# omahs/celestia-app

Hardware: AMD Instinct MI355X
Metric: EDS+DAH squares/sec (k=128) (higher is better)
Workload: dtype u8; 1 GPU; k=128 ODS -> EDS + 4k NMT roots + DAH, batch replay; k=128, field=GF(2^8), parallelism=batch1, input_layout=ODS in Q0 of the EDS buffer (placed by the upload), batches_in_flight=4

## Files before the change

### celestia-app_amd/csrc/nmt_device.hpp

```cpp
#pragma once
#include <hip/hip_runtime.h>

#include "cel_internal.hpp"
#include "sha256_device.hpp"

namespace cel {

__device__ __forceinline__ void load_node(const uint32_t* p, uint32_t (&n)[kNodeWords]) {
  const uint4* q = reinterpret_cast<const uint4*>(p);
#pragma unroll
  for (int i = 0; i < 6; i++) {
    const uint4 v = q[i];
    n[4 * i] = v.x; n[4 * i + 1] = v.y; n[4 * i + 2] = v.z; n[4 * i + 3] = v.w;
  }
}

__device__ __forceinline__ void store_node(uint32_t* p, const uint32_t (&n)[kNodeWords]) {
  uint4* q = reinterpret_cast<uint4*>(p);
#pragma unroll
  for (int i = 0; i < 6; i++) q[i] = make_uint4(n[4 * i], n[4 * i + 1], n[4 * i + 2], n[4 * i + 3]);
}

__device__ __forceinline__ void put_digest(uint32_t (&nd)[kNodeWords], const uint32_t (&st)[8]) {
  uint32_t sw[8];
#pragma unroll
  for (int i = 0; i < 8; i++) sw[i] = bswap32(st[i]);
  nd[14] = (nd[14] & 0xFFFFu) | (sw[0] << 16);
#pragma unroll
  for (int i = 15; i <= 21; i++) nd[i] = __builtin_amdgcn_alignbyte(sw[i - 14], sw[i - 15], 2);
  nd[22] = sw[7] >> 16;
  nd[23] = 0;
}


constexpr uint32_t kLeafParPrefix[7] = {0x00FFFFFFu, 0xFFFFFFFFu, 0xFFFFFFFFu, 0xFFFFFFFFu,
                                        0xFFFFFFFFu, 0xFFFFFFFFu, 0xFFFFFFFFu};
constexpr ShaMid kLeafParMid = sha_midstate(kLeafParPrefix, 7);

template <bool PF>
__device__ __forceinline__ void leaf_hash(uint32_t (&st)[8], const uint32_t* __restrict__ sh, bool q0) {
  sha256_init(st);
  uint32_t w[16];
  uint32_t nx[17];
  auto load17 = [&](int b) {
    const uint32_t* base = sh + 16 * b - 8;
    const uint4* p4 = reinterpret_cast<const uint4*>(base);
#pragma unroll
    for (int i = 0; i < 4; i++) {
      const uint4 v = p4[i];
      nx[4 * i] = v.x; nx[4 * i + 1] = v.y; nx[4 * i + 2] = v.z; nx[4 * i + 3] = v.w;
    }
    nx[16] = base[16];
  };
  {
    uint32_t s[9];
    const uint4* p4 = reinterpret_cast<const uint4*>(sh);
    const uint4 v0 = p4[0], v1 = p4[1];
    s[0] = v0.x; s[1] = v0.y; s[2] = v0.z; s[3] = v0.w; s[4] = v1.x; s[5] = v1.y; s[6] = v1.z; s[7] = v1.w;
    s[8] = sh[8];
    if (PF) load17(1);
#pragma unroll
    for (int i = 8; i < 16; i++) w[i] = perm(s[i - 8], s[i - 7], 0x06070001u);
    if (__all(!q0)) {
#pragma unroll
      for (int i = 0; i < 7; i++) w[i] = kLeafParPrefix[i];
      w[7] = 0xFFFF0000u | perm(0u, s[0], 0x0C0C0001u);
      sha256_compress_from<7>(st, mid_regs(kLeafParMid), w);
    } else {
      if (q0) {
        w[0] = perm(0u, s[0], 0x0C000102u);
#pragma unroll
        for (int i = 1; i < 7; i++) w[i] = perm(s[i - 1], s[i], 0x07000102u);
        w[7] = perm(s[6], s[7], 0x07000C0Cu) | perm(0u, s[0], 0x0C0C0001u);
      } else {
#pragma unroll
        for (int i = 0; i < 7; i++) w[i] = kLeafParPrefix[i];
        w[7] = 0xFFFF0000u | perm(0u, s[0], 0x0C0C0001u);
      }
      sha256_compress(st, w);
    }
  }
#pragma unroll 1
  for (int b = 1; b < 8; b++) {
    if (!PF) load17(b);
#pragma unroll
    for (int i = 0; i < 16; i++) w[i] = perm(nx[i], nx[i + 1], 0x06070001u);
    if (PF) {
      if (b < 7) {
        load17(b + 1);
      } else {
        const uint4* p4 = reinterpret_cast<const uint4*>(sh + 120);
        const uint4 v0 = p4[0], v1 = p4[1];
        nx[0] = v0.x; nx[1] = v0.y; nx[2] = v0.z; nx[3] = v0.w; nx[4] = v1.x; nx[5] = v1.y; nx[6] = v1.z; nx[7] = v1.w;
      }
    }
    sha256_compress(st, w);
  }
  {
    if (!PF) {
      const uint4* p4 = reinterpret_cast<const uint4*>(sh + 120);
      const uint4 v0 = p4[0], v1 = p4[1];
      nx[0] = v0.x; nx[1] = v0.y; nx[2] = v0.z; nx[3] = v0.w; nx[4] = v1.x; nx[5] = v1.y; nx[6] = v1.z; nx[7] = v1.w;
    }
#pragma unroll
    for (int i = 0; i < 7; i++) w[i] = perm(nx[i], nx[i + 1], 0x06070001u);
    w[7] = perm(nx[7], 0x80u, 0x0607000Cu);
#pragma unroll
    for (int i = 8; i < 15; i++) w[i] = 0u;
    w[15] = 542u * 8u;
    sha256_compress(st, w);
  }
}

__device__ __forceinline__ void leaf_record(const uint32_t* __restrict__ sh, bool q0, const uint32_t (&st)[8],
                                            uint32_t (&nd)[kNodeWords]) {
  if (q0) {
    const uint4* p4 = reinterpret_cast<const uint4*>(sh);
    uint32_t s[8];
    const uint4 v0 = p4[0], v1 = p4[1];
    s[0] = v0.x; s[1] = v0.y; s[2] = v0.z; s[3] = v0.w; s[4] = v1.x; s[5] = v1.y; s[6] = v1.z; s[7] = v1.w;
#pragma unroll
    for (int i = 0; i < 7; i++) nd[i] = s[i];
    nd[7] = (s[7] & 0xFFu) | (s[0] << 8);
#pragma unroll
    for (int i = 0; i < 6; i++) nd[8 + i] = __builtin_amdgcn_alignbyte(s[i + 1], s[i], 3);
    nd[14] = (s[6] >> 24) | ((s[7] & 0xFFu) << 8);
  } else {
#pragma unroll
    for (int i = 0; i < 14; i++) nd[i] = 0xFFFFFFFFu;
    nd[14] = 0xFFFFu;
  }
  put_digest(nd, st);
}

template <bool PF>
__device__ __forceinline__ void make_leaf_node(const uint32_t* __restrict__ sh, bool q0, uint32_t (&nd)[kNodeWords]) {
  uint32_t st[8];
  leaf_hash<PF>(st, sh, q0);
  leaf_record(sh, q0, st, nd);
}

__device__ __forceinline__ bool ns_less(const uint32_t* __restrict__ a, const uint32_t* __restrict__ b) {
  const uint4* pa = reinterpret_cast<const uint4*>(a);
  const uint4* pb = reinterpret_cast<const uint4*>(b);
  uint32_t x[8], y[8];
#pragma unroll
  for (int i = 0; i < 2; i++) {
    const uint4 u = pa[i], v = pb[i];
    x[4 * i] = u.x; x[4 * i + 1] = u.y; x[4 * i + 2] = u.z; x[4 * i + 3] = u.w;
    y[4 * i] = v.x; y[4 * i + 1] = v.y; y[4 * i + 2] = v.z; y[4 * i + 3] = v.w;
  }
  int res = 0;
#pragma unroll
  for (int i = 0; i < 8; i++) {
    uint32_t xa = bswap32(x[i]), yb = bswap32(y[i]);
    if (i == 7) { xa &= 0xFF000000u; yb &= 0xFF000000u; }
    if (res == 0 && xa != yb) res = xa < yb ? -1 : 1;
  }
  return res < 0;
}

__device__ __forceinline__ bool min_is_parity(const uint32_t* __restrict__ R) {
  bool par = (R[7] & 0xFFu) == 0xFFu;
#pragma unroll
  for (int q = 0; q < 7; q++) par = par && (R[q] == 0xFFFFFFFFu);
  return par;
}


constexpr uint32_t kNodeParPrefix[14] = {0x01FFFFFFu, 0xFFFFFFFFu, 0xFFFFFFFFu, 0xFFFFFFFFu, 0xFFFFFFFFu,
                                         0xFFFFFFFFu, 0xFFFFFFFFu, 0xFFFFFFFFu, 0xFFFFFFFFu, 0xFFFFFFFFu,
                                         0xFFFFFFFFu, 0xFFFFFFFFu, 0xFFFFFFFFu, 0xFFFFFFFFu};
constexpr ShaMid kNodeParMid = sha_midstate(kNodeParPrefix, 14);

__device__ __forceinline__ uint32_t node_word(const uint32_t (&L)[kNodeWords], const uint32_t (&R)[kNodeWords], int q) {
  if (q == 0) return perm(1u, L[0], 0x04000102u);
  if (q <= 21) return perm(L[q - 1], L[q], 0x07000102u);
  if (q == 22) return perm(L[21], L[22], 0x0700010Cu) | (R[0] & 0xFFu);
  if (q <= 44) return perm(R[q - 23], R[q - 22], 0x05060700u);
  if (q == 45) return perm(R[22], 0x80u, 0x05000C0Cu);
  if (q == 47) return 181u * 8u;
  return 0u;
}

__device__ __forceinline__ void hash_node(const uint32_t (&L)[kNodeWords], const uint32_t (&R)[kNodeWords],
                                          uint32_t (&out)[kNodeWords]) {
  uint32_t st[8];
  sha256_init(st);
  bool lpar = (L[14] & 0xFFFFu) == 0xFFFFu;
#pragma unroll
  for (int i = 0; i < 14; i++) lpar = lpar && (L[i] == 0xFFFFFFFFu);
  {
    uint32_t w[16];
    if (__all(lpar)) {
#pragma unroll
      for (int wi = 0; wi < 14; wi++) w[wi] = kNodeParPrefix[wi];
      w[14] = node_word(L, R, 14);
      w[15] = node_word(L, R, 15);
      sha256_compress_from<14>(st, mid_regs(kNodeParMid), w);
    } else {
#pragma unroll
      for (int wi = 0; wi < 16; wi++) w[wi] = node_word(L, R, wi);
      sha256_compress(st, w);
    }
  }
#pragma unroll
  for (int b = 1; b < 3; b++) {
    uint32_t w[16];
#pragma unroll
    for (int wi = 0; wi < 16; wi++) w[wi] = node_word(L, R, 16 * b + wi);
    sha256_compress(st, w);
  }
  bool rpar = (R[7] & 0xFFu) == 0xFFu;
#pragma unroll
  for (int i = 0; i < 7; i++) rpar = rpar && (R[i] == 0xFFFFFFFFu);
#pragma unroll
  for (int i = 0; i < 7; i++) out[i] = L[i];
  const uint32_t X7 = rpar ? L[7] : R[7];
  out[7] = (L[7] & 0xFFu) | (X7 & 0xFFFFFF00u);
#pragma unroll
  for (int i = 8; i < 14; i++) out[i] = rpar ? L[i] : R[i];
  out[14] = (rpar ? L[14] : R[14]) & 0xFFFFu;
  put_digest(out, st);
}

__device__ __forceinline__ void hash_pair(const uint32_t* in, uint64_t li, uint64_t ri, uint32_t (&o)[kNodeWords]) {
  uint32_t L[kNodeWords], R[kNodeWords];
  load_node(in + li * kNodeWords, L);
  load_node(in + ri * kNodeWords, R);
  hash_node(L, R, o);
}


constexpr uint32_t kParNodeWords[48] = {
    0x01FFFFFFu, 0xFFFFFFFFu, 0xFFFFFFFFu, 0xFFFFFFFFu, 0xFFFFFFFFu, 0xFFFFFFFFu, 0xFFFFFFFFu, 0xFFFFFFFFu,
    0xFFFFFFFFu, 0xFFFFFFFFu, 0xFFFFFFFFu, 0xFFFFFFFFu, 0xFFFFFFFFu, 0xFFFFFFFFu, 0xFFFFFF00u, 0x00000000u,
    0x00000000u, 0x00000000u, 0x00000000u, 0x00000000u, 0x00000000u, 0x00000000u, 0x000000FFu, 0xFFFFFFFFu,
    0xFFFFFFFFu, 0xFFFFFFFFu, 0xFFFFFFFFu, 0xFFFFFFFFu, 0xFFFFFFFFu, 0xFFFFFFFFu, 0xFFFFFFFFu, 0xFFFFFFFFu,
    0xFFFFFFFFu, 0xFFFFFFFFu, 0xFFFFFFFFu, 0xFFFFFFFFu, 0xFFFFFFFFu, 0xFF000000u, 0x00000000u, 0x00000000u,
    0x00000000u, 0x00000000u, 0x00000000u, 0x00000000u, 0x00000000u, 0x00800000u, 0x00000000u, 181u * 8u};

template <bool COMPACT>
__device__ __forceinline__ void hash_parity_node(const uint32_t (&dl)[8], const uint32_t (&dr)[8],
                                                 uint32_t (&out)[8]) {
  constexpr int kEnd = COMPACT ? 32 : 64;
  uint32_t st[8], w[16];
  sha256_init(st);
  auto finish = [&](ShaRegs& r) {
    if (COMPACT) sha256_rounds_tail(r, w);
    sha256_add(st, r);
  };
  {
#pragma unroll
    for (int i = 0; i < 14; i++) w[i] = kParNodeWords[i];
    w[14] = kParNodeWords[14] | (dl[0] >> 24);
    w[15] = __builtin_amdgcn_alignbit(dl[0], dl[1], 24);
    ShaRegs r = mid_regs(kNodeParMid);
    sha256_rounds_folded<14, kEnd>(r, w);
    finish(r);
  }
  {
#pragma unroll
    for (int i = 0; i < 6; i++) w[i] = __builtin_amdgcn_alignbit(dl[i + 1], dl[i + 2], 24);
    w[6] = kParNodeWords[22] | (dl[7] << 8);
#pragma unroll
    for (int i = 7; i < 16; i++) w[i] = kParNodeWords[16 + i];
    ShaRegs r{st[0], st[1], st[2], st[3], st[4], st[5], st[6], st[7]};
    sha256_rounds_folded<0, kEnd>(r, w);
    finish(r);
  }
  {
#pragma unroll
    for (int i = 0; i < 5; i++) w[i] = kParNodeWords[32 + i];
    w[5] = kParNodeWords[37] | (dr[0] >> 8);
#pragma unroll
    for (int i = 6; i < 13; i++) w[i] = __builtin_amdgcn_alignbit(dr[i - 6], dr[i - 5], 8);
    w[13] = kParNodeWords[45] | (dr[7] << 24);
    w[14] = kParNodeWords[46];
    w[15] = kParNodeWords[47];
    ShaRegs r{st[0], st[1], st[2], st[3], st[4], st[5], st[6], st[7]};
    sha256_rounds_folded<0, kEnd>(r, w);
    finish(r);
  }
#pragma unroll
  for (int i = 0; i < 8; i++) out[i] = st[i];
}

__device__ __forceinline__ void parity_record(const uint32_t (&d)[8], uint32_t (&nd)[kNodeWords]) {
#pragma unroll
  for (int i = 0; i < 14; i++) nd[i] = 0xFFFFFFFFu;
  nd[14] = 0xFFFFu;
  put_digest(nd, d);
}

__device__ __forceinline__ void load_digest(const uint32_t* p, uint32_t (&d)[8]) {
  const uint4* q = reinterpret_cast<const uint4*>(p);
  const uint4 a = q[0], b = q[1];
  d[0] = a.x; d[1] = a.y; d[2] = a.z; d[3] = a.w; d[4] = b.x; d[5] = b.y; d[6] = b.z; d[7] = b.w;
}

__device__ __forceinline__ void store_digest(uint32_t* p, const uint32_t (&d)[8]) {
  uint4* q = reinterpret_cast<uint4*>(p);
  q[0] = make_uint4(d[0], d[1], d[2], d[3]);
  q[1] = make_uint4(d[4], d[5], d[6], d[7]);
}


__device__ __forceinline__ void sha_empty(uint32_t (&st)[8]) {
  uint32_t w[16];
  w[0] = 0x80000000u;
#pragma unroll
  for (int i = 1; i < 16; i++) w[i] = 0;
  sha256_init(st);
  sha256_compress(st, w);
}

__device__ __forceinline__ void rfc_leaf90(const uint32_t (&R)[kNodeWords], uint32_t (&st)[8]) {
  sha256_init(st);
#pragma unroll
  for (int b = 0; b < 2; b++) {
    uint32_t w[16];
#pragma unroll
    for (int wi = 0; wi < 16; wi++) {
      const int q = 16 * b + wi;
      uint32_t x;
      if (q == 0) x = perm(0u, R[0], 0x0C000102u);
      else if (q <= 21) x = perm(R[q - 1], R[q], 0x07000102u);
      else if (q == 22) x = perm(R[21], R[22], 0x0700010Cu) | 0x80u;
      else if (q == 31) x = 91u * 8u;
      else x = 0u;
      w[wi] = x;
    }
    sha256_compress(st, w);
  }
}

__device__ __forceinline__ void rfc_inner(const uint32_t* l, const uint32_t* r, uint32_t (&st)[8]) {
  uint32_t w[16];
  w[0] = 0x01000000u | (l[0] >> 8);
#pragma unroll
  for (int i = 1; i < 8; i++) w[i] = __builtin_amdgcn_alignbit(l[i - 1], l[i], 8);
  w[8] = __builtin_amdgcn_alignbit(l[7], r[0], 8);
#pragma unroll
  for (int i = 9; i < 16; i++) w[i] = __builtin_amdgcn_alignbit(r[i - 9], r[i - 8], 8);
  sha256_init(st);
  uint32_t w2[16];
  w2[0] = (r[7] << 24) | 0x00800000u;
#pragma unroll
  for (int i = 1; i < 15; i++) w2[i] = 0;
  w2[15] = 65u * 8u;
  sha256_compress(st, w);
  sha256_compress(st, w2);
}

}
```

### celestia-app_amd/csrc/nmt_kernels.hip

```cpp
#include <hip/hip_runtime.h>

#include <climits>

#include "cel_internal.hpp"
#include "nmt_device.hpp"
#include "nmt_host.hpp"
#include "sha256_device.hpp"

namespace cel {




template <bool ORDER, bool PF>
__global__ __launch_bounds__(256) void k_leaf(const uint8_t* __restrict__ eds, uint32_t k, uint32_t* __restrict__ leaves,
                                              int32_t* __restrict__ bad_axis, uint32_t cell0, uint32_t cell1) {
  const uint32_t W = 2 * k;
  const uint32_t cell = cell0 + blockIdx.x * 256u + threadIdx.x;
  if (cell >= cell1) return;
  const uint32_t r = cell / W, c = cell % W;
  const uint64_t sq_eds = (uint64_t)W * W * kShare;
  const uint32_t* sh = reinterpret_cast<const uint32_t*>(eds + blockIdx.y * sq_eds + (uint64_t)cell * kShare);
  const bool q0 = (r < k) && (c < k);
  {
    uint32_t nd[kNodeWords];
    make_leaf_node<PF>(sh, q0, nd);
    store_node(leaves + ((uint64_t)blockIdx.y * W * W + cell) * kNodeWords, nd);
  }
  __builtin_amdgcn_sched_barrier(0);
  if (ORDER && q0) {
    if (c > 0 && ns_less(sh, sh - kShare / 4)) atomicMin(bad_axis + blockIdx.y, (int32_t)r);
    if (r > 0 && ns_less(sh, sh - (uint64_t)W * kShare / 4)) atomicMin(bad_axis + blockIdx.y, (int32_t)(W + c));
  }
}


__device__ __forceinline__ void put_root(const uint32_t (&o)[kNodeWords], uint32_t sq, uint32_t t, uint32_t W,
                                         uint32_t* __restrict__ leafd, uint8_t* __restrict__ row_out,
                                         uint8_t* __restrict__ col_out) {
  {
    uint8_t* r = (t < W ? row_out + ((uint64_t)sq * W + t) * kNode : col_out + ((uint64_t)sq * W + (t - W)) * kNode);
    uint16_t* r16 = reinterpret_cast<uint16_t*>(r);
#pragma unroll
    for (int i = 0; i < 45; i++) r16[i] = (uint16_t)(o[i / 2] >> (16 * (i & 1)));
  }
  if (leafd) {
    uint32_t st[8];
    rfc_leaf90(o, st);
    uint4* d = reinterpret_cast<uint4*>(leafd + ((uint64_t)sq * 2 * W + t) * 8);
    d[0] = make_uint4(st[0], st[1], st[2], st[3]);
    d[1] = make_uint4(st[4], st[5], st[6], st[7]);
  }
}

template <bool FROM_LEAVES>
__global__ __launch_bounds__(256) void k_level(const uint32_t* __restrict__ in, uint32_t* __restrict__ out, uint32_t W,
                                               uint32_t nin, uint32_t trees, uint32_t* __restrict__ leafd,
                                               uint8_t* __restrict__ row_out, uint8_t* __restrict__ col_out) {
  const uint32_t nout = nin / 2;
  const uint32_t idx = blockIdx.x * 256u + threadIdx.x;
  if (idx >= trees * nout) return;
  const uint32_t t = idx / nout, j = idx % nout;
  uint64_t li, ri;
  if (FROM_LEAVES) {
    const uint64_t sq = (uint64_t)blockIdx.y * W * W;
    if (t < W) { li = sq + (uint64_t)t * W + 2 * j; ri = li + 1; }
    else { li = sq + (uint64_t)(2 * j) * W + (t - W); ri = li + W; }
  } else {
    const uint64_t sq = (uint64_t)blockIdx.y * trees * nin;
    li = sq + (uint64_t)t * nin + 2 * j;
    ri = li + 1;
  }
  uint32_t o[kNodeWords];
  hash_pair(in, li, ri, o);
  const uint64_t oi = (uint64_t)blockIdx.y * trees * nout + idx;
  store_node(out + oi * kNodeWords, o);
  if (row_out) put_root(o, blockIdx.y, t, W, leafd, row_out, col_out);
}


__host__ __device__ constexpr uint32_t q_nodes(uint32_t k, uint32_t n) { return k * n; }
__host__ __device__ constexpr uint32_t p_nodes(uint32_t k, uint32_t n) { return 3 * k * n; }
__device__ __forceinline__ uint32_t q_node(uint32_t k, uint32_t n, uint32_t t, uint32_t i) {
  return (t < k ? t : t - k) * (n / 2) + i;
}
__device__ __forceinline__ uint32_t p_node(uint32_t k, uint32_t n, uint32_t t, uint32_t i) {
  const uint32_t W = 2 * k, a = t < W ? t : t - W;
  if (a < k) return (t < W ? a : k + a) * (n / 2) + (i - n / 2);
  return k * n + (t < W ? a - k : a) * n + i;
}

template <bool ROOT>
__global__ __launch_bounds__(256) void k_level_split(const uint32_t* __restrict__ qin, uint32_t* __restrict__ qout,
                                                     const uint32_t* __restrict__ pin, uint32_t* __restrict__ pout,
                                                     uint32_t nq, uint32_t np, uint32_t bq, uint32_t k,
                                                     uint32_t* __restrict__ leafd, uint8_t* __restrict__ row_out,
                                                     uint8_t* __restrict__ col_out) {
  const uint32_t sq = blockIdx.y, W = 2 * k;
  if (blockIdx.x < bq) {
    const uint32_t i = blockIdx.x * 256u + threadIdx.x;
    if (i >= nq) return;
    uint32_t o[kNodeWords];
    if (ROOT) {
      uint32_t L[kNodeWords], R[kNodeWords], d[8];
      load_node(qin + ((uint64_t)sq * nq + i) * kNodeWords, L);
      load_digest(pin + ((uint64_t)sq * 3 * np + i) * 8, d);
      parity_record(d, R);
      hash_node(L, R, o);
      put_root(o, sq, i < k ? i : W + (i - k), W, leafd, row_out, col_out);
    } else {
      hash_pair(qin + (uint64_t)sq * 2 * nq * kNodeWords, 2 * i, 2 * i + 1, o);
      store_node(qout + ((uint64_t)sq * nq + i) * kNodeWords, o);
    }
  } else {
    const uint32_t i = (blockIdx.x - bq) * 256u + threadIdx.x;
    if (i >= np) return;
    const uint32_t* in = pin + (ROOT ? (uint64_t)sq * 3 * np + np : (uint64_t)sq * 2 * np) * 8;
    uint32_t dl[8], dr[8], d[8];
    load_digest(in + (uint64_t)i * 16, dl);
    load_digest(in + (uint64_t)i * 16 + 8, dr);
    hash_parity_node<false>(dl, dr, d);
    if (ROOT) {
      uint32_t o[kNodeWords];
      parity_record(d, o);
      put_root(o, sq, i < k ? k + i : W + i, W, leafd, row_out, col_out);
    } else {
      store_digest(pout + ((uint64_t)sq * np + i) * 8, d);
    }
  }
}


template <bool ORDER, bool PF, bool ROOTS>
__global__ __launch_bounds__(256) __attribute__((amdgpu_waves_per_eu(3, 3))) void k_leaf_quad(
    const uint8_t* __restrict__ eds, uint32_t k, uint32_t* __restrict__ out, uint32_t* __restrict__ pout,
    int32_t* __restrict__ bad_axis, uint32_t* __restrict__ leafd, uint8_t* __restrict__ row_out,
    uint8_t* __restrict__ col_out) {
  const uint32_t W = 2 * k, trees = 2 * W;
  const uint32_t tw = k < 8 ? k : 8u, th = 64 / tw, tiles_x = k / tw;
  const uint32_t g = blockIdx.x * 256u + threadIdx.x, tile = g / 64, l = g % 64;
  const uint32_t bi = (tile / tiles_x) * th + l / tw, bj = (tile % tiles_x) * tw + l % tw;
  if (bi >= k) return;
  const uint64_t sq_eds = (uint64_t)W * W * kShare;
  const uint32_t* sh00 =
      reinterpret_cast<const uint32_t*>(eds + blockIdx.y * sq_eds + ((uint64_t)(2 * bi) * W + 2 * bj) * kShare);
  uint32_t dA[8], dB[8], dC[8];
#pragma unroll 1
  for (uint32_t s = 0; s < 4; s++) {
    const uint32_t r = 2 * bi + (s >> 1), c = 2 * bj + (s & 1);
    const uint32_t* sh = sh00 + ((uint64_t)(s >> 1) * W + (s & 1)) * (kShare / 4);
    const bool q0 = (r < k) && (c < k);
    {
      uint32_t st[8];
      leaf_hash<PF>(st, sh, q0);
#pragma unroll
      for (int i = 0; i < 8; i++) {
        if (s == 0 || s == 3) dA[i] = st[i];
        if (s == 1) dB[i] = st[i];
        if (s == 2) dC[i] = st[i];
      }
    }
    const uint32_t nn = s == 3 ? 2u : (s ? 1u : 0u);
#pragma unroll 1
    for (uint32_t n = 0; n < nn; n++) {
      const uint32_t lc = s < 3 ? 0u : 1u + n;
      const bool row = (s == 1) || (s == 3 && n == 1);
      const uint32_t* shl = sh00 + ((uint64_t)(lc >> 1) * W + (lc & 1)) * (kShare / 4);
      const bool q0l = (2 * bi + (lc >> 1) < k) && (2 * bj + (lc & 1) < k);
      const uint32_t t = row ? r : W + c, idx = row ? bj : bi;
      auto children = [&](uint32_t (&dl)[8], uint32_t (&dr)[8]) {
#pragma unroll
        for (int i = 0; i < 8; i++) {
          dl[i] = lc == 0 ? dA[i] : (lc == 1 ? dB[i] : dC[i]);
          dr[i] = s == 1 ? dB[i] : (s == 2 ? dC[i] : dA[i]);
        }
      };
      if (ROOTS || q0l) {
        uint32_t o[kNodeWords];
        {
          uint32_t L[kNodeWords], R[kNodeWords], dl[8], dr[8];
          children(dl, dr);
          leaf_record(shl, q0l, dl, L);
          leaf_record(sh, q0, dr, R);
          hash_node(L, R, o);
        }
        if (ROOTS) {
          store_node(out + (((uint64_t)blockIdx.y * trees + t) * k + idx) * kNodeWords, o);
          put_root(o, blockIdx.y, t, W, leafd, row_out, col_out);
        } else {
          store_node(out + ((uint64_t)blockIdx.y * q_nodes(k, k) + q_node(k, k, t, idx)) * kNodeWords, o);
        }
      } else {
        uint32_t dl[8], dr[8], o[8];
        children(dl, dr);
        hash_parity_node<true>(dl, dr, o);
        store_digest(pout + ((uint64_t)blockIdx.y * p_nodes(k, k) + p_node(k, k, t, idx)) * 8, o);
      }
    }
    __builtin_amdgcn_sched_barrier(0);
    if (ORDER && q0) {
      if (c > 0 && ns_less(sh, sh - kShare / 4)) atomicMin(bad_axis + blockIdx.y, (int32_t)r);
      if (r > 0 && ns_less(sh, sh - (uint64_t)W * kShare / 4)) atomicMin(bad_axis + blockIdx.y, (int32_t)(W + c));
    }
  }
}



__global__ __launch_bounds__(1024) void k_merkle(const uint32_t* __restrict__ items, const uint32_t* __restrict__ leafd,
                                                uint32_t n, uint8_t* dah, const int32_t* __restrict__ bad_axis,
                                                int32_t* status, const uint8_t* out_src,
                                                uint8_t* __restrict__ host_out, uint32_t out_bytes) {
  extern __shared__ __attribute__((aligned(16))) uint32_t hs[];
  const uint32_t g = blockIdx.x;
  const uint32_t* it = items + (uint64_t)g * n * kNodeWords;
  if (leafd) {
    for (uint32_t i = threadIdx.x; i < n * 8; i += blockDim.x) hs[i] = leafd[(uint64_t)g * n * 8 + i];
  } else {
    for (uint32_t i = threadIdx.x; i < n; i += blockDim.x) {
      uint32_t R[kNodeWords], st[8];
      load_node(it + (uint64_t)i * kNodeWords, R);
      rfc_leaf90(R, st);
#pragma unroll
      for (int j = 0; j < 8; j++) hs[i * 8 + j] = st[j];
    }
  }
  __syncthreads();
  uint32_t cnt = n;
  while (cnt > 1) {
    const uint32_t half = cnt / 2;
    uint32_t st[8];
    for (uint32_t base = 0; base < half; base += blockDim.x) {
      const uint32_t i = base + threadIdx.x;
      if (i < half) rfc_inner(hs + (2 * i) * 8, hs + (2 * i + 1) * 8, st);
      __syncthreads();
      if (i < half) {
#pragma unroll
        for (int j = 0; j < 8; j++) hs[i * 8 + j] = st[j];
      }
      __syncthreads();
    }
    if (cnt & 1) {
      if (threadIdx.x < 8) hs[half * 8 + threadIdx.x] = hs[(cnt - 1) * 8 + threadIdx.x];
      __syncthreads();
    }
    cnt = half + (cnt & 1);
  }
  if (threadIdx.x == 0) {
    uint32_t st[8];
    if (n == 0) sha_empty(st);
    else
      for (int j = 0; j < 8; j++) st[j] = hs[j];
    for (int j = 0; j < 8; j++) {
      dah[g * 32 + 4 * j] = (uint8_t)(st[j] >> 24);
      dah[g * 32 + 4 * j + 1] = (uint8_t)(st[j] >> 16);
      dah[g * 32 + 4 * j + 2] = (uint8_t)(st[j] >> 8);
      dah[g * 32 + 4 * j + 3] = (uint8_t)st[j];
    }
    if (status) status[g] = (bad_axis && bad_axis[g] != INT_MAX) ? CEL_EORDER : CEL_OK;
  }
  if (host_out) {
    __threadfence();
    __syncthreads();
    const uint4* src = reinterpret_cast<const uint4*>(out_src);
    uint4* dst = reinterpret_cast<uint4*>(host_out);
    for (uint32_t i = threadIdx.x; i < out_bytes / 16; i += blockDim.x) dst[i] = src[i];
  }
}

static uint32_t merkle_block(uint32_t n) {
  const uint32_t pairs = ((n / 2 + 63) / 64) * 64;
  return pairs < 64 ? 64u : (pairs > 1024 ? 1024u : pairs);
}

__global__ __launch_bounds__(256) void k_dah_leaves(const uint32_t* __restrict__ items, uint32_t n,
                                                    uint32_t* __restrict__ leafd, uint8_t* __restrict__ row_out,
                                                    uint8_t* __restrict__ col_out) {
  const uint32_t i = blockIdx.x * 256u + threadIdx.x;
  if (i >= n) return;
  uint32_t R[kNodeWords], st[8];
  load_node(items + (uint64_t)i * kNodeWords, R);
  rfc_leaf90(R, st);
  uint4* d = reinterpret_cast<uint4*>(leafd + (uint64_t)i * 8);
  d[0] = make_uint4(st[0], st[1], st[2], st[3]);
  d[1] = make_uint4(st[4], st[5], st[6], st[7]);
  const uint32_t half = n / 2;
  uint16_t* r16 = reinterpret_cast<uint16_t*>(i < half ? row_out + (uint64_t)i * kNode : col_out + (uint64_t)(i - half) * kNode);
#pragma unroll
  for (int j = 0; j < 45; j++) r16[j] = (uint16_t)(R[j / 2] >> (16 * (j & 1)));
}

__global__ void k_fill_i32(int32_t* p, uint32_t n, int32_t v) {
  const uint32_t i = blockIdx.x * blockDim.x + threadIdx.x;
  if (i < n) p[i] = v;
}


void launch_fill_i32(int32_t* p, uint32_t n, int32_t v, uint32_t block, hipStream_t s) {
  hipLaunchKernelGGL(k_fill_i32, dim3((n + block - 1) / block), dim3(block), 0, s, p, n, v);
}

void launch_dah_leaves(const uint32_t* items, uint32_t n, uint32_t* leafd, uint8_t* row_out, uint8_t* col_out,
                       hipStream_t s) {
  hipLaunchKernelGGL(k_dah_leaves, dim3((n + 255) / 256), dim3(256), 0, s, items, n, leafd, row_out, col_out);
}

void launch_merkle(const uint32_t* items, const uint32_t* leafd, uint32_t n, uint32_t lists, uint8_t* dah,
                   const int32_t* bad_axis, int32_t* status, hipStream_t s, const uint8_t* out_src, uint8_t* host_out,
                   uint32_t out_bytes) {
  const size_t lds = (size_t)(n ? n : 1) * 8 * 4;
  hipLaunchKernelGGL(k_merkle, dim3(lists), dim3(merkle_block(n)), lds, s, items, leafd, n, dah, bad_axis, status,
                     out_src, host_out, out_bytes);
}

struct CommitWork {
  uint32_t *leaves, *ping, *pong, *roots, *leafd;
  uint32_t *q[2], *p[2];
  int32_t* bad;
  size_t size;
};

static bool quad_path(uint32_t nsq) { return nsq > 1; }

static CommitWork commit_work(void* work, uint32_t k, uint32_t nsq) {
  const size_t W = 2 * (size_t)k, nb = kNodeWords * 4;
  Carver c(work);
  CommitWork w;
  w.leaves = c.take<uint32_t>(quad_path(nsq) ? 0 : nsq * W * W * nb);
  w.ping = c.take<uint32_t>(nsq * 2 * W * (W / 2 + 1) * nb);
  w.pong = c.take<uint32_t>(nsq * 2 * W * (W / 4 + 1) * nb);
  w.roots = c.take<uint32_t>(nsq * 2 * W * nb);
  w.bad = c.take<int32_t>((size_t)nsq * 4 + 4);
  w.leafd = c.take<uint32_t>(nsq * 2 * W * 32);
  w.size = c.size();
  for (uint32_t i = 0; i < 2; i++) {
    Carver a(i ? w.pong : w.ping);
    w.q[i] = a.take<uint32_t>((size_t)nsq * q_nodes(k, k >> i) * nb);
    w.p[i] = a.take<uint32_t>((size_t)nsq * p_nodes(k, k >> i) * 32);
  }
  return w;
}

size_t nmt_workspace_size(uint32_t k, uint32_t nsq) { return commit_work(nullptr, k, nsq).size; }

hipError_t launch_commit_leaves(const uint8_t* eds, uint32_t k, uint32_t nsq, void* work, bool order_check,
                                uint32_t row0, uint32_t row1, bool init_bad, hipStream_t s) {
  if (quad_path(nsq)) return hipErrorInvalidValue;
  const uint32_t W = 2 * k;
  const CommitWork w = commit_work(work, k, nsq);
  const Range r("nmt.leaf");
  if (init_bad) launch_fill_i32(w.bad, nsq, INT_MAX, 256, s);
  const uint32_t c0 = row0 * W, c1 = row1 * W;
  if (c1 <= c0) return hipGetLastError();
  dim3 gl((c1 - c0 + 255) / 256, nsq);
  dispatch_order_pf(order_check, latency_bound((uint64_t)(c1 - c0) * nsq), [&](auto order, auto pf) {
    hipLaunchKernelGGL((k_leaf<decltype(order)::value, decltype(pf)::value>), gl, dim3(256), 0, s, eds, k, w.leaves,
                       w.bad, c0, c1);
  });
  return hipGetLastError();
}

static hipError_t commit_dah(const CommitWork& w, uint32_t k, uint32_t nsq, uint8_t* row_roots, uint8_t* dah,
                             int32_t* status, hipStream_t s, uint8_t* host_out, uint32_t out_bytes) {
  const Range r("dah");
  if (dah)
    launch_merkle(w.roots, w.leafd, 4 * k, nsq, dah, w.bad, status, s, host_out ? row_roots : nullptr, host_out,
                  out_bytes);
  return hipGetLastError();
}

static hipError_t commit_levels(const CommitWork& w, uint32_t k, uint32_t nsq, uint8_t* row_roots,
                                uint8_t* col_roots, uint8_t* dah, int32_t* status, hipStream_t s, uint8_t* host_out,
                                uint32_t out_bytes) {
  const uint32_t W = 2 * k;
  const uint32_t trees = 2 * W;
  uint32_t nin = W;
  const uint32_t* src = w.leaves;
  uint32_t* dst = w.ping;
  bool first = true;
  roctxRangePushA("nmt.levels");
  while (nin > 1) {
    const uint32_t nout = nin / 2;
    uint32_t* out = (nout == 1) ? w.roots : dst;
    uint32_t* ld = (nout == 1 && dah) ? w.leafd : nullptr;
    dim3 g((trees * nout + 255) / 256, nsq);
    uint8_t* ro = (nout == 1) ? row_roots : nullptr;
    uint8_t* co = (nout == 1) ? col_roots : nullptr;
    if (first) hipLaunchKernelGGL(k_level<true>, g, dim3(256), 0, s, src, out, W, nin, trees, ld, ro, co);
    else hipLaunchKernelGGL(k_level<false>, g, dim3(256), 0, s, src, out, W, nin, trees, ld, ro, co);
    first = false;
    src = out;
    dst = (dst == w.ping) ? w.pong : w.ping;
    nin = nout;
  }
  roctxRangePop();
  return commit_dah(w, k, nsq, row_roots, dah, status, s, host_out, out_bytes);
}

hipError_t launch_commit_trees(uint32_t k, uint32_t nsq, uint8_t* row_roots, uint8_t* col_roots, uint8_t* dah,
                               int32_t* status, void* work, hipStream_t s, uint8_t* host_out, uint32_t out_bytes) {
  if (quad_path(nsq)) return hipErrorInvalidValue;
  return commit_levels(commit_work(work, k, nsq), k, nsq, row_roots, col_roots, dah, status, s, host_out, out_bytes);
}

static hipError_t launch_commit_quads(const uint8_t* eds, uint32_t k, uint32_t nsq, const CommitWork& w,
                                      bool order_check, uint8_t* row_roots, uint8_t* col_roots, bool want_dah,
                                      hipStream_t s) {
  const Range r("nmt.leaf");
  launch_fill_i32(w.bad, nsq, INT_MAX, 256, s);
  const uint32_t tw = k < 8 ? k : 8u, th = 64 / tw;
  const uint64_t lanes = (uint64_t)((k + th - 1) / th) * (k / tw) * 64;
  dim3 g((uint32_t)((lanes + 255) / 256), nsq);
  if (k == 1) {
    uint32_t* ld = want_dah ? w.leafd : nullptr;
    if (order_check)
      hipLaunchKernelGGL((k_leaf_quad<true, false, true>), g, dim3(256), 0, s, eds, k, w.roots, nullptr, w.bad, ld,
                         row_roots, col_roots);
    else
      hipLaunchKernelGGL((k_leaf_quad<false, false, true>), g, dim3(256), 0, s, eds, k, w.roots, nullptr, w.bad, ld,
                         row_roots, col_roots);
    return hipGetLastError();
  }
  dispatch_order_pf(order_check, latency_bound(lanes * nsq), [&](auto order, auto pf) {
    hipLaunchKernelGGL((k_leaf_quad<decltype(order)::value, decltype(pf)::value, false>), g, dim3(256), 0, s, eds, k,
                       w.q[0], w.p[0], w.bad, nullptr, nullptr, nullptr);
  });
  return hipGetLastError();
}

static hipError_t commit_levels_split(const CommitWork& w, uint32_t k, uint32_t nsq, uint8_t* row_roots,
                                      uint8_t* col_roots, bool want_dah, hipStream_t s) {
  const Range r("nmt.levels");
  uint32_t at = 0;
  for (uint32_t n = k; n > 2; n /= 2, at ^= 1) {
    const uint32_t nq = q_nodes(k, n / 2), np = p_nodes(k, n / 2), bq = (nq + 255) / 256;
    hipLaunchKernelGGL(k_level_split<false>, dim3(bq + (np + 255) / 256, nsq), dim3(256), 0, s, w.q[at], w.q[at ^ 1],
                       w.p[at], w.p[at ^ 1], nq, np, bq, k, nullptr, nullptr, nullptr);
  }
  const uint32_t nr = 2 * k, bq = (nr + 255) / 256;
  hipLaunchKernelGGL(k_level_split<true>, dim3(2 * bq, nsq), dim3(256), 0, s, w.q[at], nullptr, w.p[at], nullptr, nr,
                     nr, bq, k, want_dah ? w.leafd : nullptr, row_roots, col_roots);
  return hipGetLastError();
}

hipError_t launch_commit(const uint8_t* eds, uint32_t k, uint32_t nsq, uint8_t* row_roots, uint8_t* col_roots,
                         uint8_t* dah, int32_t* status, void* work, bool order_check, hipStream_t s) {
  if (!quad_path(nsq)) {
    hipError_t e = launch_commit_leaves(eds, k, nsq, work, order_check, 0, 2 * k, true, s);
    if (e == hipSuccess) e = launch_commit_trees(k, nsq, row_roots, col_roots, dah, status, work, s);
    return e;
  }
  const CommitWork w = commit_work(work, k, nsq);
  hipError_t e = launch_commit_quads(eds, k, nsq, w, order_check, row_roots, col_roots, dah != nullptr, s);
  if (e == hipSuccess && k > 1) e = commit_levels_split(w, k, nsq, row_roots, col_roots, dah != nullptr, s);
  if (e == hipSuccess) e = commit_dah(w, k, nsq, row_roots, dah, status, s, nullptr, 0);
  return e;
}


}
```

Baseline: 22990 squares/s.

## Split leaf-quad kernel into Q0-only and parity-only launches with specialized hashing

The leaf-level quad kernel is split into two launches. One covers only Q0 tiles, the other only the parity tiles, so each lane's cell type is known at compile time. This removes the per-lane q0 checks and the wave-wide __all votes on parity prefixes, and lets parity blocks always use the precomputed SHA midstate. The cost is an extra kernel launch and code duplication; small k keeps the old path.

```diff
diff --git a/celestia-app_amd/csrc/nmt_device.hpp b/celestia-app_amd/csrc/nmt_device.hpp
--- a/celestia-app_amd/csrc/nmt_device.hpp
+++ b/celestia-app_amd/csrc/nmt_device.hpp
@@ -37,8 +37,11 @@
                                         0xFFFFFFFFu, 0xFFFFFFFFu, 0xFFFFFFFFu};
 constexpr ShaMid kLeafParMid = sha_midstate(kLeafParPrefix, 7);
 
-template <bool PF>
+enum class Cells { kAny, kQ0, kParity };
+
+template <bool PF, Cells C = Cells::kAny>
 __device__ __forceinline__ void leaf_hash(uint32_t (&st)[8], const uint32_t* __restrict__ sh, bool q0) {
+  if (C != Cells::kAny) q0 = C == Cells::kQ0;
   sha256_init(st);
   uint32_t w[16];
   uint32_t nx[17];
@@ -61,7 +64,7 @@
     if (PF) load17(1);
 #pragma unroll
     for (int i = 8; i < 16; i++) w[i] = perm(s[i - 8], s[i - 7], 0x06070001u);
-    if (__all(!q0)) {
+    if (C == Cells::kParity || (C == Cells::kAny && __all(!q0))) {
 #pragma unroll
       for (int i = 0; i < 7; i++) w[i] = kLeafParPrefix[i];
       w[7] = 0xFFFF0000u | perm(0u, s[0], 0x0C0C0001u);
@@ -183,16 +186,17 @@
   return 0u;
 }
 
+template <bool PAR_START = true>
 __device__ __forceinline__ void hash_node(const uint32_t (&L)[kNodeWords], const uint32_t (&R)[kNodeWords],
                                           uint32_t (&out)[kNodeWords]) {
   uint32_t st[8];
   sha256_init(st);
-  bool lpar = (L[14] & 0xFFFFu) == 0xFFFFu;
+  bool lpar = PAR_START && (L[14] & 0xFFFFu) == 0xFFFFu;
 #pragma unroll
   for (int i = 0; i < 14; i++) lpar = lpar && (L[i] == 0xFFFFFFFFu);
   {
     uint32_t w[16];
-    if (__all(lpar)) {
+    if (PAR_START && __all(lpar)) {
 #pragma unroll
       for (int wi = 0; wi < 14; wi++) w[wi] = kNodeParPrefix[wi];
       w[14] = node_word(L, R, 14);
diff --git a/celestia-app_amd/csrc/nmt_kernels.hip b/celestia-app_amd/csrc/nmt_kernels.hip
--- a/celestia-app_amd/csrc/nmt_kernels.hip
+++ b/celestia-app_amd/csrc/nmt_kernels.hip
@@ -5,6 +5,7 @@
 #include "cel_internal.hpp"
 #include "nmt_device.hpp"
 #include "nmt_host.hpp"
+#include "quad_tiles.hpp"
 #include "sha256_device.hpp"
 
 namespace cel {
@@ -131,28 +132,26 @@
 }
 
 
-template <bool ORDER, bool PF, bool ROOTS>
-__global__ __launch_bounds__(256) __attribute__((amdgpu_waves_per_eu(3, 3))) void k_leaf_quad(
-    const uint8_t* __restrict__ eds, uint32_t k, uint32_t* __restrict__ out, uint32_t* __restrict__ pout,
-    int32_t* __restrict__ bad_axis, uint32_t* __restrict__ leafd, uint8_t* __restrict__ row_out,
-    uint8_t* __restrict__ col_out) {
+template <Cells C, bool ORDER, bool PF, bool ROOTS>
+__device__ __forceinline__ void quad_block(const uint8_t* __restrict__ eds, uint32_t k, uint32_t sq, uint32_t bi,
+                                           uint32_t bj, uint32_t* __restrict__ out, uint32_t* __restrict__ pout,
+                                           int32_t* __restrict__ bad_axis, uint32_t* __restrict__ leafd,
+                                           uint8_t* __restrict__ row_out, uint8_t* __restrict__ col_out) {
+  static_assert(C == Cells::kAny || !ROOTS, "the roots case is a mixed block");
   const uint32_t W = 2 * k, trees = 2 * W;
-  const uint32_t tw = k < 8 ? k : 8u, th = 64 / tw, tiles_x = k / tw;
-  const uint32_t g = blockIdx.x * 256u + threadIdx.x, tile = g / 64, l = g % 64;
-  const uint32_t bi = (tile / tiles_x) * th + l / tw, bj = (tile % tiles_x) * tw + l % tw;
-  if (bi >= k) return;
   const uint64_t sq_eds = (uint64_t)W * W * kShare;
   const uint32_t* sh00 =
-      reinterpret_cast<const uint32_t*>(eds + blockIdx.y * sq_eds + ((uint64_t)(2 * bi) * W + 2 * bj) * kShare);
+      reinterpret_cast<const uint32_t*>(eds + sq * sq_eds + ((uint64_t)(2 * bi) * W + 2 * bj) * kShare);
+  auto in_q0 = [&](uint32_t r, uint32_t c) { return C == Cells::kAny ? (r < k) && (c < k) : C == Cells::kQ0; };
   uint32_t dA[8], dB[8], dC[8];
 #pragma unroll 1
   for (uint32_t s = 0; s < 4; s++) {
     const uint32_t r = 2 * bi + (s >> 1), c = 2 * bj + (s & 1);
     const uint32_t* sh = sh00 + ((uint64_t)(s >> 1) * W + (s & 1)) * (kShare / 4);
-    const bool q0 = (r < k) && (c < k);
+    const bool q0 = in_q0(r, c);
     {
       uint32_t st[8];
-      leaf_hash<PF>(st, sh, q0);
+      leaf_hash<PF, C>(st, sh, q0);
 #pragma unroll
       for (int i = 0; i < 8; i++) {
         if (s == 0 || s == 3) dA[i] = st[i];
@@ -166,7 +165,7 @@
       const uint32_t lc = s < 3 ? 0u : 1u + n;
       const bool row = (s == 1) || (s == 3 && n == 1);
       const uint32_t* shl = sh00 + ((uint64_t)(lc >> 1) * W + (lc & 1)) * (kShare / 4);
-      const bool q0l = (2 * bi + (lc >> 1) < k) && (2 * bj + (lc & 1) < k);
+      const bool q0l = in_q0(2 * bi + (lc >> 1), 2 * bj + (lc & 1));
       const uint32_t t = row ? r : W + c, idx = row ? bj : bi;
       auto children = [&](uint32_t (&dl)[8], uint32_t (&dr)[8]) {
 #pragma unroll
@@ -182,27 +181,63 @@
           children(dl, dr);
           leaf_record(shl, q0l, dl, L);
           leaf_record(sh, q0, dr, R);
-          hash_node(L, R, o);
+          hash_node<C == Cells::kAny>(L, R, o);
         }
         if (ROOTS) {
-          store_node(out + (((uint64_t)blockIdx.y * trees + t) * k + idx) * kNodeWords, o);
-          put_root(o, blockIdx.y, t, W, leafd, row_out, col_out);
+          store_node(out + (((uint64_t)sq * trees + t) * k + idx) * kNodeWords, o);
+          put_root(o, sq, t, W, leafd, row_out, col_out);
         } else {
-          store_node(out + ((uint64_t)blockIdx.y * q_nodes(k, k) + q_node(k, k, t, idx)) * kNodeWords, o);
+          store_node(out + ((uint64_t)sq * q_nodes(k, k) + q_node(k, k, t, idx)) * kNodeWords, o);
         }
       } else {
         uint32_t dl[8], dr[8], o[8];
         children(dl, dr);
-        hash_parity_node<true>(dl, dr, o);
-        store_digest(pout + ((uint64_t)blockIdx.y * p_nodes(k, k) + p_node(k, k, t, idx)) * 8, o);
+        hash_parity_node<C == Cells::kAny>(dl, dr, o);
+        store_digest(pout + ((uint64_t)sq * p_nodes(k, k) + p_node(k, k, t, idx)) * 8, o);
       }
     }
     __builtin_amdgcn_sched_barrier(0);
     if (ORDER && q0) {
-      if (c > 0 && ns_less(sh, sh - kShare / 4)) atomicMin(bad_axis + blockIdx.y, (int32_t)r);
-      if (r > 0 && ns_less(sh, sh - (uint64_t)W * kShare / 4)) atomicMin(bad_axis + blockIdx.y, (int32_t)(W + c));
-    }
-  }
+      if (c > 0 && ns_less(sh, sh - kShare / 4)) atomicMin(bad_axis + sq, (int32_t)r);
+      if (r > 0 && ns_less(sh, sh - (uint64_t)W * kShare / 4)) atomicMin(bad_axis + sq, (int32_t)(W + c));
+    }
+  }
+}
+
+template <bool ORDER, bool PF, bool ROOTS>
+__global__ __launch_bounds__(256) __attribute__((amdgpu_waves_per_eu(3, 3))) void k_leaf_quad(
+    const uint8_t* __restrict__ eds, uint32_t k, uint32_t* __restrict__ out, uint32_t* __restrict__ pout,
+    int32_t* __restrict__ bad_axis, uint32_t* __restrict__ leafd, uint8_t* __restrict__ row_out,
+    uint8_t* __restrict__ col_out) {
+  const uint32_t tw = k < 8 ? k : 8u, th = 64 / tw, tiles_x = k / tw;
+  const uint32_t g = blockIdx.x * 256u + threadIdx.x, tile = g / 64, l = g % 64;
+  const uint32_t bi = (tile / tiles_x) * th + l / tw, bj = (tile % tiles_x) * tw + l % tw;
+  if (bi >= k) return;
+  quad_block<Cells::kAny, ORDER, PF, ROOTS>(eds, k, blockIdx.y, bi, bj, out, pout, bad_axis, leafd, row_out, col_out);
+}
+
+template <bool ORDER, bool PF>
+__global__ __launch_bounds__(256) __attribute__((amdgpu_waves_per_eu(3, 3))) void k_leaf_quad_q0(
+    const uint8_t* __restrict__ eds, uint32_t k, uint32_t* __restrict__ out, int32_t* __restrict__ bad_axis) {
+  const uint32_t g = blockIdx.x * quad::kGroupLanes + threadIdx.x;
+  const uint32_t tile = g / quad::kTileLanes, l = g % quad::kTileLanes;
+  if (tile >= quad::q0_tiles(k)) return;
+  const quad::TilePos at = quad::q0_tile(tile, k);
+  quad_block<Cells::kQ0, ORDER, PF, false>(eds, k, blockIdx.y, at.row * quad::kTileSide + l / quad::kTileSide,
+                                           at.col * quad::kTileSide + l % quad::kTileSide, out, nullptr, bad_axis,
+                                           nullptr, nullptr, nullptr);
+}
+
+template <bool PF>
+__global__ __launch_bounds__(256) __attribute__((amdgpu_waves_per_eu(3, 3))) void k_leaf_quad_par(
+    const uint8_t* __restrict__ eds, uint32_t k, uint32_t* __restrict__ pout) {
+  const uint32_t g = blockIdx.x * quad::kGroupLanes + threadIdx.x;
+  const uint32_t tile = g / quad::kTileLanes, l = g % quad::kTileLanes;
+  if (tile >= quad::par_tiles(k)) return;
+  const quad::TilePos at = quad::par_tile(tile, k);
+  quad_block<Cells::kParity, false, PF, false>(eds, k, blockIdx.y, at.row * quad::kTileSide + l / quad::kTileSide,
+                                               at.col * quad::kTileSide + l % quad::kTileSide, nullptr, pout, nullptr,
+                                               nullptr, nullptr, nullptr);
 }
 
 
@@ -421,9 +456,21 @@
                          row_roots, col_roots);
     return hipGetLastError();
   }
-  dispatch_order_pf(order_check, latency_bound(lanes * nsq), [&](auto order, auto pf) {
-    hipLaunchKernelGGL((k_leaf_quad<decltype(order)::value, decltype(pf)::value, false>), g, dim3(256), 0, s, eds, k,
-                       w.q[0], w.p[0], w.bad, nullptr, nullptr, nullptr);
+  if (!quad::split_width(k)) {
+    dispatch_order_pf(order_check, latency_bound(lanes * nsq), [&](auto order, auto pf) {
+      hipLaunchKernelGGL((k_leaf_quad<decltype(order)::value, decltype(pf)::value, false>), g, dim3(256), 0, s, eds,
+                         k, w.q[0], w.p[0], w.bad, nullptr, nullptr, nullptr);
+    });
+    return hipGetLastError();
+  }
+  const uint32_t gq = quad::groups_for(quad::q0_tiles(k)), gp = quad::groups_for(quad::par_tiles(k));
+  dispatch_order_pf(order_check, latency_bound((uint64_t)gq * quad::kGroupLanes * nsq), [&](auto order, auto pf) {
+    hipLaunchKernelGGL((k_leaf_quad_q0<decltype(order)::value, decltype(pf)::value>), dim3(gq, nsq),
+                       dim3(quad::kGroupLanes), 0, s, eds, k, w.q[0], w.bad);
+  });
+  dispatch_order_pf(false, latency_bound((uint64_t)gp * quad::kGroupLanes * nsq), [&](auto, auto pf) {
+    hipLaunchKernelGGL((k_leaf_quad_par<decltype(pf)::value>), dim3(gp, nsq), dim3(quad::kGroupLanes), 0, s, eds, k,
+                       w.p[0]);
   });
   return hipGetLastError();
 }
diff --git a/celestia-app_amd/csrc/quad_tiles.hpp b/celestia-app_amd/csrc/quad_tiles.hpp
--- /dev/null
+++ b/celestia-app_amd/csrc/quad_tiles.hpp
@@ -0,0 +1,44 @@
+#pragma once
+#include <cstdint>
+
+#ifdef __HIPCC__
+#define CEL_TILE_HD __host__ __device__
+#else
+#define CEL_TILE_HD
+#endif
+
+namespace cel {
+namespace quad {
+
+constexpr uint32_t kTileSide = 8;
+constexpr uint32_t kTileLanes = kTileSide * kTileSide;
+constexpr uint32_t kGroupLanes = 256;
+constexpr uint32_t kMinSplitK = 2 * kTileSide;
+
+struct TilePos {
+  uint32_t row, col;
+};
+
+CEL_TILE_HD constexpr bool split_width(uint32_t k) { return k >= kMinSplitK && k % kMinSplitK == 0; }
+
+CEL_TILE_HD constexpr uint32_t q0_tiles(uint32_t k) { return (k / 16) * (k / 16); }
+CEL_TILE_HD constexpr uint32_t par_tiles(uint32_t k) { return 3 * (k / 16) * (k / 16); }
+
+CEL_TILE_HD constexpr TilePos q0_tile(uint32_t i, uint32_t k) {
+  const uint32_t h = k / 16;
+  return TilePos{i / h, i % h};
+}
+
+CEL_TILE_HD constexpr TilePos par_tile(uint32_t i, uint32_t k) {
+  const uint32_t h = k / 16;
+  if (i < h * h) return TilePos{i / h, h + i % h};
+  const uint32_t j = i - h * h;
+  return TilePos{h + j / (2 * h), j % (2 * h)};
+}
+
+CEL_TILE_HD constexpr uint32_t groups_for(uint32_t tiles) {
+  return (tiles * kTileLanes + kGroupLanes - 1) / kGroupLanes;
+}
+
+}
+}
```

New measurement: 23470 squares/s (median of 6 runs). +2.1%, better.
